# deepomicslab/PALACE

Measured on AMD Instinct MI355X. Metric: contigs/sec eref+generate_graph+matching, 1M-contig synth, 1/2/4/8 GPU, higher is better.
Workload: dtype u32

## Files before the change

palace_amd/csrc/common.hpp:

```cpp
#pragma once
#include <hip/hip_runtime.h>
#include <cstdarg>
#include <cstdint>
#include <cstdio>
#include <cstring>
#include <vector>

#include "../../include/palace_hip.h"

namespace palace {

void set_error(const char *fmt, ...);

#define PALACE_HIP_TRY(expr)                                                                    \
    do {                                                                                        \
        hipError_t e__ = (expr);                                                                \
        if (e__ != hipSuccess) {                                                                \
            palace::set_error("%s failed: %s (%s:%d)", #expr, hipGetErrorString(e__), __FILE__, \
                              __LINE__);                                                        \
            return PALACE_EHIP;                                                                 \
        }                                                                                       \
    } while (0)

#define PALACE_REQUIRE(cond, msg)                                  \
// ... 11 lines not shown

struct CoderMasks {
    uint32_t m[3][3];
};

struct Workspace {
    void *ptr = nullptr;
    size_t bytes = 0;
};

}

namespace palace {
struct MatchScratch;
void free_match_scratch(MatchScratch *m);
}

struct palace_ctx {
    int device = 0;
    hipStream_t stream = nullptr;
    bool owns_stream = true;
    hipEvent_t ev0 = nullptr, ev1 = nullptr;
    uint32_t key_buckets[4] = {~0u, ~0u, ~0u, ~0u};
    std::vector<hipEvent_t> marks;
    bool coder_set = false;
    palace::CoderMasks masks{};
    uint32_t *plane[3] = {nullptr, nullptr, nullptr};
    bool planes_external = false;
    bool want_final = false;
    bool final_only = false;
    bool table_clean = false;
    int64_t keys_counted = 0;
    const struct palace_eref_probe_index *probe_ix = nullptr;
    const struct palace_eref_probe_index *c0_hits_ix = nullptr;
    uint32_t hits_mask = 0;
    int probe_all_sets = 0;
    bool sent_scattered = false;
    int64_t scan_ref_lo = 0, scan_ref_hi = 0;
    const void *counts_ptr = nullptr;
    bool planeless = false;
    int count_mode = 0;
    int64_t bin_cap_override = 0;
    int64_t slab_override = 0;
    palace::Workspace ws;
    bool ws_grown = false;
    palace::Workspace pin;
    palace::MatchScratch *match_scratch = nullptr;
    int64_t graph_border = -1;
    const void *graph_border_cands = nullptr;
    int64_t graph_border_n = -1;
    int match_grid = 0;
    bool match_two_word_keys = false;
    int match_iters = 0;
    uint64_t *d_small = nullptr;
};

namespace palace {
int ensure_workspace(palace_ctx *ctx, size_t bytes);
int ensure_pinned(palace_ctx *ctx, size_t bytes);
int ensure_table(palace_ctx *ctx);
}
```

palace_amd/csrc/decomp.hip:

```cpp
#include "decomp.hpp"

#include <algorithm>

namespace palace {

namespace {

constexpr uint64_t kNoKey = ~0ull;
constexpr uint64_t kClosed = 0;
constexpr int kStampShift = 42;
constexpr int kPackedShift = 52, kPackedStamps = 1 << (64 - kPackedShift);
constexpr uint64_t kLenMask = (1ull << 40) - 1;


__device__ __forceinline__ uint64_t wave_incl_scan(uint64_t v, int lane)
{
#pragma unroll
    for (int d = 1; d < 64; d <<= 1) {
        const uint64_t u = __shfl_up(v, d);
        if (lane >= d) v += u;
    }
    return v;
}

constexpr int kMaxWaves = 16;

__device__ void scan_partials_body(const uint64_t *__restrict__ in, int64_t n, uint64_t *__restrict__ partials, int blk, int nblk)
{
    __shared__ uint64_t part[kMaxWaves];
    const int64_t chunk = (n + nblk - 1) / nblk;
    const int64_t a = min(n, static_cast<int64_t>(blk) * chunk), e = min(n, a + chunk);
    uint64_t s = 0;
    for (int64_t i = a + threadIdx.x; i < e; i += blockDim.x) s += in[i];
    const int lane = threadIdx.x & 63, waves = static_cast<int>(blockDim.x >> 6);
    s = wave_incl_scan(s, lane);
    if (lane == 63) part[threadIdx.x >> 6] = s;
    __syncthreads();
    if (threadIdx.x == 0) {
        uint64_t t = 0;
        for (int w = 0; w < waves; w++) t += part[w];
        partials[blk] = t;
    }
    __syncthreads();
}

__device__ void scan_prefix_body(uint64_t *__restrict__ partials, int n_parts, uint64_t *__restrict__ total)
{
    __shared__ uint64_t part[kMaxWaves];
    const int lane = threadIdx.x & 63, wv = threadIdx.x >> 6;
    const uint64_t x = static_cast<int>(threadIdx.x) < n_parts ? partials[threadIdx.x] : 0;
    const uint64_t incl = wave_incl_scan(x, lane);
    if (lane == 63) part[wv] = incl;
    __syncthreads();
    uint64_t before = 0;
    for (int w = 0; w < wv; w++) before += part[w];
    if (static_cast<int>(threadIdx.x) < n_parts) partials[threadIdx.x] = before + incl - x;
    if (threadIdx.x == blockDim.x - 1) *total = before + incl;
    __syncthreads();
}

__device__ void scan_apply_body(const uint64_t *__restrict__ in, uint64_t *__restrict__ out, int64_t n, const uint64_t *__restrict__ partials,
                                int blk, int nblk)
{
    __shared__ uint64_t part[kMaxWaves];
    const int64_t chunk = (n + nblk - 1) / nblk;
    const int64_t a = min(n, static_cast<int64_t>(blk) * chunk), e = min(n, a + chunk);
    const int lane = threadIdx.x & 63, wv = threadIdx.x >> 6, waves = static_cast<int>(blockDim.x >> 6);
    uint64_t carry = partials[blk];
    for (int64_t base = a; base < e; base += blockDim.x) {
        const int64_t i = base + threadIdx.x;
        const uint64_t x = i < e ? in[i] : 0;
        const uint64_t incl = wave_incl_scan(x, lane);
        if (lane == 63) part[wv] = incl;
        __syncthreads();
        uint64_t before = 0, all = 0;
        for (int w = 0; w < waves; w++) { if (w < wv) before += part[w]; all += part[w]; }
        if (i < e) out[i] = carry + before + incl - x;
        carry += all;
        __syncthreads();
    }
}

__global__ __launch_bounds__(kDecompBlock) void scan_partials_kernel(const uint64_t *__restrict__ in, const int32_t *__restrict__ n_dev,
                                                                     uint64_t *__restrict__ partials)
{
    scan_partials_body(in, *n_dev, partials, static_cast<int>(blockIdx.x), static_cast<int>(gridDim.x));
}
__global__ __launch_bounds__(kDecompBlock) void scan_prefix_kernel(uint64_t *__restrict__ partials, int n_parts, uint64_t *__restrict__ total)
{
    scan_prefix_body(partials, n_parts, total);
}
__global__ __launch_bounds__(kDecompBlock) void scan_apply_kernel(const uint64_t *__restrict__ in, uint64_t *__restrict__ out,
                                                                  const int32_t *__restrict__ n_dev, const uint64_t *__restrict__ partials)
{
    scan_apply_body(in, out, *n_dev, partials, static_cast<int>(blockIdx.x), static_cast<int>(gridDim.x));
}

struct Span { int tid, n; };
__device__ __forceinline__ Span whole_grid() { return Span{static_cast<int>(blockIdx.x * blockDim.x + threadIdx.x), static_cast<int>(gridDim.x * blockDim.x)}; }

__device__ void ph_init(const DecompBufs &b, Span T, int64_t comp_cap, int64_t vert_cap, int n_flags, int allow_packed)
{
    DecompState *st = b.st;
    const int V = st->V;
    for (int i = T.tid; i < V; i += T.n) { b.bo_hi[i] = kNoKey; b.bi_hi[i] = kNoKey; b.on_path[i] = 0; }
    for (int i = T.tid; i < n_flags; i += T.n) b.changed[i] = 0;
    if (T.tid == 0) {
        st->n_comp = 0; st->n_vert = 0; st->comp_cap = comp_cap; st->vert_cap = vert_cap;
        st->unsettled = 0; st->overflow = 0; st->bad = 0; st->dead = 0; st->scan_total = 0; st->alive_after = 0;
        st->packed = (allow_packed && b.kc && b.pack_bad && *b.pack_bad == 0) ? 1u : 0u;
        if (comp_cap >= 0) b.o_off[0] = 0;
    }
}

__device__ void ph_round_begin(const DecompBufs &b, Span T, int reset_left)
{
    const int V = b.st->V;
    if (!reset_left && b.st->dead) return;
    if (T.tid == 0) { b.st->alive_after = 0; if (reset_left) b.st->dead = 0; }
    const int64_t E = b.st->E;
    for (int64_t e = T.tid; e < E; e += T.n) b.done[e] = 0;
    const bool packed = b.st->packed != 0;
    for (int i = T.tid; i < V; i += T.n) {
        const int s = i >> 1;
        const int64_t l = reset_left ? 1 : b.left[s];
        if (reset_left && !(i & 1)) b.left[s] = 1;
        b.alive[i] = l > 0;
        b.next[i] = -1; b.prev[i] = -1;
        b.bo_hi[i] = b.bi_hi[i] = l > 0 ? kNoKey : kClosed;
        if (!packed) { b.bo_lo[i] = kNoKey; b.bo_lo[V + i] = kNoKey; b.bi_lo[i] = kNoKey; b.bi_lo[V + i] = kNoKey; }
        b.len_a[i] = 0;
    }
}

struct IterArgs {
    uint64_t stamp;
    uint64_t stamp_p;
    int parity;
    int prev_flag, flag;
    int unique_hi;
};


__device__ void ph_propose_hi(const DecompBufs &b, Span T, const IterArgs &a)
{
    if (b.st->dead) return;
    if (a.prev_flag >= 0 && !b.changed[a.prev_flag]) return;
    const int64_t E = b.st->E;
    const int V = b.st->V;
    const int other = (a.parity ^ 1) * V;
    const bool packed = b.st->packed != 0;
    for (int64_t e = T.tid; e < E; e += T.n) {
        if (b.done[e]) continue;
        const int u = b.src[e], v = b.dst[e];
        if (b.bi_hi[v] == kClosed) { b.done[e] = 1; continue; }
        const uint64_t k = packed ? (a.stamp_p | b.kc[e]) : (a.stamp | b.khi[e]);
        if (atomicMin(reinterpret_cast<unsigned long long *>(&b.bo_hi[u]), static_cast<unsigned long long>(k)) == kClosed) { b.done[e] = 1; continue; }
        atomicMin(reinterpret_cast<unsigned long long *>(&b.bi_hi[v]), static_cast<unsigned long long>(k));
        if (!a.unique_hi && !packed) { b.bo_lo[other + u] = kNoKey; b.bi_lo[other + v] = kNoKey; }
    }
}

__device__ void ph_propose_lo(const DecompBufs &b, Span T, const IterArgs &a)
{
    if (b.st->dead) return;
    if (a.prev_flag >= 0 && !b.changed[a.prev_flag]) return;
    if (b.st->packed) return;
    const int64_t E = b.st->E;
    const int mine = a.parity * b.st->V;
    for (int64_t e = T.tid; e < E; e += T.n) {
        if (b.done[e]) continue;
        const int u = b.src[e], v = b.dst[e];
        const uint64_t k = a.stamp | b.khi[e], lo = b.klo[e];
        if (b.bo_hi[u] == k) atomicMin(reinterpret_cast<unsigned long long *>(&b.bo_lo[mine + u]), static_cast<unsigned long long>(lo));
        if (b.bi_hi[v] == k) atomicMin(reinterpret_cast<unsigned long long *>(&b.bi_lo[mine + v]), static_cast<unsigned long long>(lo));
    }
}

__device__ void ph_commit_flag(const DecompBufs &b, Span T, const IterArgs &a, volatile unsigned int *took);
__device__ void ph_commit(const DecompBufs &b, Span T, const IterArgs &a)
{
    if (b.st->dead) return;
    if (a.prev_flag >= 0 && !b.changed[a.prev_flag]) return;
    ph_commit_flag(b, T, a, b.changed + a.flag);
}
__device__ void ph_commit_flag(const DecompBufs &b, Span T, const IterArgs &a, volatile unsigned int *took)
{
    bool any = false;
    const int64_t E = b.st->E;
    const int mine = a.parity * b.st->V;
    const bool packed = b.st->packed != 0;
    for (int64_t e = T.tid; e < E; e += T.n) {
        if (b.done[e]) continue;
        const int u = b.src[e], v = b.dst[e];
        const uint64_t k = packed ? (a.stamp_p | b.kc[e]) : (a.stamp | b.khi[e]);
        if (b.bo_hi[u] != k || b.bi_hi[v] != k) continue;
        const uint64_t lo = b.klo[e];
        if (!a.unique_hi && !packed && (b.bo_lo[mine + u] != lo || b.bi_lo[mine + v] != lo)) continue;
        b.next[u] = v; b.prev[v] = u;
        b.nhi[u] = b.khi[e]; b.nlo[u] = lo;
        b.bo_hi[u] = kClosed; b.bi_hi[v] = kClosed;
        b.done[e] = 1;
        any = true;
    }
    if (__syncthreads_or(any) && threadIdx.x == 0) *took = 1u;
}

__device__ void ph_heads(const DecompBufs &b, Span T, int round, int last_flag)
{
    DecompState *st = b.st;
    if (st->dead) return;
    if (T.tid == 0 && last_flag >= 0 && b.changed[last_flag]) st->unsettled = 1;
    const int V = st->V;
    for (int v = T.tid; v < V; v += T.n) {
        if (!b.alive[v] || b.prev[v] >= 0) continue;
        int len = 0, last = v;
        int64_t least = b.left[v >> 1];
        for (int x = v; x >= 0; x = b.next[x]) {
            b.on_path[x] = round + 1;
            last = x;
            len++;
            least = min(least, b.left[x >> 1]);
        }
        const int twin_first = last ^ 1;
        if (v > twin_first) continue;
        const int64_t uses = twin_first == v ? 2 : 1;
        b.len_a[v] = (1ull << 40) | static_cast<uint64_t>(len);
        b.pay[v] = max(static_cast<int64_t>(1), least / uses);
        b.kind[v] = 0;
        b.open_at[v] = 0;
    }
}

__device__ void ph_cycles(const DecompBufs &b, Span T, int round)
{
    const int V = b.st->V;
    if (b.st->dead) return;
    for (int v = T.tid; v < V; v += T.n) {
        if (!b.alive[v] || b.on_path[v] == round + 1) continue;
        int len = 1, twin_least = v ^ 1, worst = 0;
        uint64_t whi = b.nhi[v], wlo = b.nlo[v];
        int64_t least = b.left[v >> 1];
        bool first = true;
        for (int x = b.next[v]; x != v; x = b.next[x]) {
            if (x < v) { first = false; break; }
            twin_least = min(twin_least, x ^ 1);
            const uint64_t hi = b.nhi[x], lo = b.nlo[x];
            if (hi > whi || (hi == whi && lo > wlo)) { whi = hi; wlo = lo; worst = len; }
            least = min(least, b.left[x >> 1]);
            len++;
        }
        if (!first || v > twin_least) continue;
        const int64_t uses = twin_least == v ? 2 : 1;
        b.len_a[v] = (1ull << 40) | static_cast<uint64_t>(len);
        b.pay[v] = max(static_cast<int64_t>(1), least / uses);
        b.kind[v] = 1;
        b.open_at[v] = (worst + 1) % len;
    }
}

__device__ void ph_emit(const DecompBufs &b, Span T, int round, int64_t c0, int64_t v0)
{
    DecompState *st = b.st;
    const int V = st->V;
    if (st->dead) return;
    int64_t alive = 0;
    for (int v = T.tid; v < V; v += T.n) {
        const uint64_t la = b.len_a[v];
        if (!la) continue;
        const int64_t len = static_cast<int64_t>(la & kLenMask);
        const uint64_t p = b.pos[v];
        const int64_t c = c0 + static_cast<int64_t>(p >> 40), at = v0 + static_cast<int64_t>(p & kLenMask);
        const int64_t pay = b.pay[v];
        const bool room = c < st->comp_cap && at + len <= st->vert_cap;
        if (!room) st->overflow = 1;
        else { b.o_off[c] = at; b.o_kind[c] = b.kind[v]; b.o_iter[c] = round; b.o_open[c] = b.open_at[v]; }
        int x = v;
        int64_t still = 0;
        for (int64_t k = 0; k < len; k++) {
            if (room) b.o_verts[at + k] = 2 * b.orig[x >> 1] + (x & 1);
            const int64_t l = b.left[x >> 1];
            b.left[x >> 1] = max(static_cast<int64_t>(0), l - pay);
            still += l - pay > 0;
            x = b.next[x];
        }
        alive += still;
    }
    __shared__ unsigned long long wg_alive;
    if (threadIdx.x == 0) wg_alive = 0;
    __syncthreads();
    if (alive) atomicAdd(&wg_alive, static_cast<unsigned long long>(alive));
    __syncthreads();
    if (threadIdx.x == 0 && wg_alive) atomicAdd(reinterpret_cast<unsigned long long *>(&st->alive_after), wg_alive);
}


__global__ void dec_init_kernel(DecompBufs b, int64_t comp_cap, int64_t vert_cap, int n_flags, int allow_packed) { ph_init(b, whole_grid(), comp_cap, vert_cap, n_flags, allow_packed); }
__global__ void dec_round_begin_kernel(DecompBufs b, int reset_left) { ph_round_begin(b, whole_grid(), reset_left); }
__global__ void dec_propose_hi_kernel(DecompBufs b, IterArgs a) { ph_propose_hi(b, whole_grid(), a); }
__global__ void dec_propose_lo_kernel(DecompBufs b, IterArgs a) { ph_propose_lo(b, whole_grid(), a); }
__global__ void dec_commit_kernel(DecompBufs b, IterArgs a) { ph_commit(b, whole_grid(), a); }
__global__ void dec_heads_kernel(DecompBufs b, int round, int last_flag) { ph_heads(b, whole_grid(), round, last_flag); }
__global__ void dec_cycles_kernel(DecompBufs b, int round) { ph_cycles(b, whole_grid(), round); }
__global__ void dec_emit_kernel(DecompBufs b, int round) { ph_emit(b, whole_grid(), round, b.st->n_comp, b.st->n_vert); }

__global__ void dec_round_end_kernel(DecompBufs b)
{
    DecompState *st = b.st;
    if (blockIdx.x || threadIdx.x || st->dead) return;
    st->dead = st->alive_after == 0;
    st->n_comp += static_cast<int64_t>(st->scan_total >> 40);
    st->n_vert += static_cast<int64_t>(st->scan_total & kLenMask);
    if (st->n_comp <= st->comp_cap) b.o_off[st->n_comp] = st->n_vert;
}

size_t up256(size_t v) { return (v + 255) / 256 * 256; }

struct Carver {
    char *base;
    size_t used = 0;
    template <class T>
    T *take(size_t n)
    {
        T *p = base ? reinterpret_cast<T *>(base + used) : nullptr;
        used += up256(std::max<size_t>(1, n) * sizeof(T));
        return p;
    }
};

size_t carve_all(DecompBufs &b, char *base, int64_t s_cap, int64_t e_cap, int64_t comp_cap, int64_t vert_cap, int rounds, int iters)
{
    Carver c{base};
    const size_t S = static_cast<size_t>(std::max<int64_t>(1, s_cap)), V = 2 * S, E = static_cast<size_t>(std::max<int64_t>(1, e_cap));
    b.st = c.take<DecompState>(1);
    b.src = c.take<int32_t>(E); b.dst = c.take<int32_t>(E);
    b.khi = c.take<uint64_t>(E); b.klo = c.take<uint64_t>(E);
    b.done = c.take<uint8_t>(E);
    b.kc = c.take<uint64_t>(E);
    b.left = c.take<int64_t>(S); b.orig = c.take<int32_t>(S);
    b.next = c.take<int32_t>(V); b.prev = c.take<int32_t>(V); b.on_path = c.take<int32_t>(V); b.open_at = c.take<int32_t>(V);
    b.nhi = c.take<uint64_t>(V); b.nlo = c.take<uint64_t>(V);
    b.bo_hi = c.take<uint64_t>(V); b.bi_hi = c.take<uint64_t>(V);
    b.bo_lo = c.take<uint64_t>(2 * V); b.bi_lo = c.take<uint64_t>(2 * V);
    b.len_a = c.take<uint64_t>(V); b.pos = c.take<uint64_t>(V);
    b.pay = c.take<int64_t>(V);
    b.alive = c.take<uint8_t>(V); b.kind = c.take<uint8_t>(V);
    b.partials = c.take<uint64_t>(kDecompGrid + 1);
    b.changed = c.take<uint32_t>(static_cast<size_t>(rounds) * static_cast<size_t>(iters));
    b.o_off = c.take<int64_t>(static_cast<size_t>(comp_cap) + 1);
    b.o_verts = c.take<int32_t>(static_cast<size_t>(vert_cap));
    b.o_iter = c.take<int32_t>(static_cast<size_t>(comp_cap));
    b.o_open = c.take<int32_t>(static_cast<size_t>(comp_cap));
    b.o_kind = c.take<uint8_t>(static_cast<size_t>(comp_cap));
    return c.used;
}

}

size_t decomp_bytes(int64_t s_cap, int64_t e_cap, int64_t comp_cap, int64_t vert_cap, int rounds, int iters)
{
    DecompBufs tmp;
    return carve_all(tmp, nullptr, s_cap, e_cap, comp_cap, vert_cap, rounds, iters);
}

void decomp_carve(DecompBufs &b, char *base, int64_t s_cap, int64_t e_cap, int64_t comp_cap, int64_t vert_cap, int rounds, int iters)
{
    carve_all(b, base, s_cap, e_cap, comp_cap, vert_cap, rounds, iters);
}

int scan_u64(palace_ctx *ctx, const uint64_t *in, uint64_t *out, const int32_t *n_dev, uint64_t *partials, uint64_t *total_dev)
{
    hipLaunchKernelGGL(scan_partials_kernel, dim3(kDecompGrid), dim3(kDecompBlock), 0, ctx->stream, in, n_dev, partials);
    hipLaunchKernelGGL(scan_prefix_kernel, dim3(1), dim3(kDecompBlock), 0, ctx->stream, partials, kDecompGrid, total_dev);
    hipLaunchKernelGGL(scan_apply_kernel, dim3(kDecompGrid), dim3(kDecompBlock), 0, ctx->stream, in, out, n_dev, partials);
    PALACE_HIP_TRY(hipGetLastError());
    return PALACE_OK;
}

namespace {

const dim3 kBlock(kDecompBlock);
constexpr int kWideGridDefault = 2048;
inline dim3 wide_grid(const palace_ctx *ctx) { return dim3(ctx->match_grid > 0 ? ctx->match_grid : kWideGridDefault); }

void enqueue_iterations(palace_ctx *ctx, const DecompBufs &b, int first, int n, uint64_t *count, int flag0, bool unique_hi)
{
    for (int k = 0; k < n; k++) {
        IterArgs a{((1ull << 21) - 1 - *count) << kStampShift, static_cast<uint64_t>((kPackedStamps - 1 - *count) & (kPackedStamps - 1)) << kPackedShift,
                   (first + k) & 1, k ? flag0 + k - 1 : -1, flag0 + k, unique_hi ? 1 : 0};
        (*count)++;
        hipLaunchKernelGGL(dec_propose_hi_kernel, wide_grid(ctx), kBlock, 0, ctx->stream, b, a);
        if (!unique_hi) hipLaunchKernelGGL(dec_propose_lo_kernel, wide_grid(ctx), kBlock, 0, ctx->stream, b, a);
        hipLaunchKernelGGL(dec_commit_kernel, wide_grid(ctx), kBlock, 0, ctx->stream, b, a);
    }
}

int enqueue_read_off(palace_ctx *ctx, const DecompBufs &b, int round, int last_flag)
{
    hipLaunchKernelGGL(dec_heads_kernel, wide_grid(ctx), kBlock, 0, ctx->stream, b, round, last_flag);
    hipLaunchKernelGGL(dec_cycles_kernel, wide_grid(ctx), kBlock, 0, ctx->stream, b, round);
    int rc = scan_u64(ctx, b.len_a, b.pos, &b.st->V, b.partials, &b.st->scan_total);
    if (rc) return rc;
    hipLaunchKernelGGL(dec_emit_kernel, wide_grid(ctx), kBlock, 0, ctx->stream, b, round);
    hipLaunchKernelGGL(dec_round_end_kernel, dim3(1), dim3(64), 0, ctx->stream, b);
    PALACE_HIP_TRY(hipGetLastError());
    return PALACE_OK;
}

}

int decomp_begin(palace_ctx *ctx, const DecompBufs &b, int rounds, int64_t comp_cap, int64_t vert_cap)
{
    PALACE_REQUIRE(rounds >= 1 && rounds <= kMaxRounds, "round count out of range");
    static_assert(kDecompGrid <= kDecompBlock, "scan_prefix_kernel scans the block sums with one workgroup");
    const int allow_packed = !ctx->match_two_word_keys && static_cast<int64_t>(rounds) * kMaxIters < kPackedStamps ? 1 : 0;
    hipLaunchKernelGGL(dec_init_kernel, wide_grid(ctx), kBlock, 0, ctx->stream, b, comp_cap, vert_cap, rounds * kMaxIters, allow_packed);
    PALACE_HIP_TRY(hipGetLastError());
    return PALACE_OK;
}

int decomp_rounds(palace_ctx *ctx, const DecompBufs &b, int t0, int t1, int rounds, int aggressive, int iters, bool unique_hi,
                  uint64_t *count)
{
    PALACE_REQUIRE(0 <= t0 && t0 <= t1 && t1 <= rounds && rounds <= kMaxRounds && iters >= 1 && iters <= kMaxIters, "round / iteration count out of range");
    for (int t = t0; t < t1; t++) {
        hipLaunchKernelGGL(dec_round_begin_kernel, wide_grid(ctx), kBlock, 0, ctx->stream, b, (aggressive && t == rounds - 1) ? 1 : 0);
        enqueue_iterations(ctx, b, 0, iters, count, t * kMaxIters, unique_hi);
        int rc = enqueue_read_off(ctx, b, t, t * kMaxIters + iters - 1);
        if (rc) return rc;
    }
    PALACE_HIP_TRY(hipGetLastError());
    return PALACE_OK;
}

int decomp_run_checked(palace_ctx *ctx, const DecompBufs &b, int rounds, int aggressive, bool unique_hi, int64_t comp_cap,
                       int64_t vert_cap, int64_t max_iterations)
{
    PALACE_REQUIRE(rounds >= 1 && rounds <= kMaxRounds, "round count out of range");
    constexpr int kBatch = 16;
    hipLaunchKernelGGL(dec_init_kernel, wide_grid(ctx), kBlock, 0, ctx->stream, b, comp_cap, vert_cap, kBatch, 0);
    uint64_t count = 0;
    for (int t = 0; t < rounds; t++) {
        hipLaunchKernelGGL(dec_round_begin_kernel, wide_grid(ctx), kBlock, 0, ctx->stream, b, (aggressive && t == rounds - 1) ? 1 : 0);
        for (int first = 0;; first += kBatch) {
            PALACE_HIP_TRY(hipMemsetAsync(b.changed, 0, kBatch * sizeof(uint32_t), ctx->stream));
            enqueue_iterations(ctx, b, first, kBatch, &count, 0, unique_hi);
            uint32_t last = 0;
            PALACE_HIP_TRY(hipMemcpyAsync(&last, b.changed + kBatch - 1, sizeof last, hipMemcpyDeviceToHost, ctx->stream));
            PALACE_HIP_TRY(hipStreamSynchronize(ctx->stream));
            if (!last) break;
            if (static_cast<int64_t>(count) > max_iterations || count + kBatch >= (1ull << 21)) {
                set_error("matching: no fixed point after %llu iterations", static_cast<unsigned long long>(count));
                return PALACE_ESTATE;
            }
        }
        PALACE_HIP_TRY(hipMemsetAsync(b.changed, 0, kBatch * sizeof(uint32_t), ctx->stream));
        int rc = enqueue_read_off(ctx, b, t, kBatch - 1);
        if (rc) return rc;
    }
    return PALACE_OK;
}

int decomp_group(palace_ctx *ctx, const DecompBufs &b, DecompRun &run, int rounds, int aggressive, bool unique_hi)
{
    const int first = kFirstGroupRounds;
    const int t0 = run.next_round, t1 = std::min(rounds, t0 + (t0 == 0 ? first : kRoundsPerGroup));
    for (int t = t0; t < t1; t++) {
        const int iters = ctx->match_iters > 0 ? std::min(ctx->match_iters, kMaxIters) : (t == 0 ? kFirstRoundIters : kLaterRoundIters);
        int rc = decomp_rounds(ctx, b, t, t + 1, rounds, aggressive, iters, unique_hi, &run.count);
        if (rc) return rc;
    }
    run.next_round = t1;
    return PALACE_OK;
}

int decomp_finish(palace_ctx *ctx, const DecompBufs &b, DecompRun &run, int rounds, int aggressive, bool unique_hi, int64_t comp_cap,
                  int64_t vert_cap, int64_t max_iterations, DecompState *h_state, const std::function<int()> &reset_left)
{
    for (;;) {
        PALACE_HIP_TRY(hipMemcpyAsync(h_state, b.st, sizeof *h_state, hipMemcpyDeviceToHost, ctx->stream));
        PALACE_HIP_TRY(hipStreamSynchronize(ctx->stream));
        if (h_state->unsettled) {
            int rc = reset_left();
            if (rc) return rc;
            rc = decomp_run_checked(ctx, b, rounds, aggressive, unique_hi, comp_cap, vert_cap, max_iterations);
            if (rc) return rc;
            PALACE_HIP_TRY(hipMemcpyAsync(h_state, b.st, sizeof *h_state, hipMemcpyDeviceToHost, ctx->stream));
            PALACE_HIP_TRY(hipStreamSynchronize(ctx->stream));
            return PALACE_OK;
        }
        if (run.next_round >= rounds) return PALACE_OK;
        if (h_state->alive_after == 0) {
            if (!aggressive) return PALACE_OK;
            run.next_round = rounds - 1;
        }
        int rc = decomp_group(ctx, b, run, rounds, aggressive, unique_hi);
        if (rc) return rc;
    }
}

}
```

palace_amd/csrc/decomp.hpp:

```cpp
#pragma once
#include <functional>

#include "common.hpp"

struct palace_match_result {
    int64_t n = 0;
    int64_t *off = nullptr;
    int32_t *verts = nullptr, *iter = nullptr, *open_at = nullptr;
    uint8_t *kind = nullptr;
    uint64_t *bare = nullptr;
    int64_t n_bare = 0;
    bool borrowed = false;
    ~palace_match_result();
};

namespace palace {

constexpr int kDecompGrid = 256;
constexpr int kDecompBlock = 256;
constexpr int kMaxRounds = 1024;
constexpr int kMaxIters = 64;

struct DecompState {
    int32_t S, V;
    int64_t E;
    int64_t n_comp, n_vert;
    int64_t comp_cap, vert_cap;
    uint32_t unsettled;
    uint32_t overflow;
    uint32_t bad;
    uint32_t dead;
    uint32_t packed;
    uint64_t scan_total;
    int64_t alive_after;
};

struct DecompBufs {
    DecompState *st = nullptr;
    int32_t *src = nullptr, *dst = nullptr;
    uint64_t *khi = nullptr, *klo = nullptr;
    uint8_t *done = nullptr;
    uint64_t *kc = nullptr;
    const uint32_t *pack_bad = nullptr;
    int64_t *left = nullptr;
    int32_t *orig = nullptr;
    int32_t *next = nullptr, *prev = nullptr, *on_path = nullptr, *open_at = nullptr;
    uint64_t *nhi = nullptr, *nlo = nullptr;
    uint64_t *bo_hi = nullptr, *bi_hi = nullptr;
    uint64_t *bo_lo = nullptr, *bi_lo = nullptr;
    uint64_t *len_a = nullptr, *pos = nullptr;
    int64_t *pay = nullptr;
    uint8_t *alive = nullptr, *kind = nullptr;
    uint64_t *partials = nullptr;
    uint32_t *changed = nullptr;
    int64_t *o_off = nullptr;
    int32_t *o_verts = nullptr, *o_iter = nullptr, *o_open = nullptr;
    uint8_t *o_kind = nullptr;
};

size_t decomp_bytes(int64_t s_cap, int64_t e_cap, int64_t comp_cap, int64_t vert_cap, int rounds, int iters);
void decomp_carve(DecompBufs &b, char *base, int64_t s_cap, int64_t e_cap, int64_t comp_cap, int64_t vert_cap, int rounds, int iters);
constexpr int kFirstRoundIters = 7, kLaterRoundIters = 4, kRoundsPerGroup = 5, kFirstGroupRounds = 5;
int decomp_begin(palace_ctx *ctx, const DecompBufs &b, int rounds, int64_t comp_cap, int64_t vert_cap);
int decomp_rounds(palace_ctx *ctx, const DecompBufs &b, int t0, int t1, int rounds, int aggressive, int iters, bool unique_hi,
                  uint64_t *count);

struct DecompRun { int next_round = 0; uint64_t count = 0; };
int decomp_group(palace_ctx *ctx, const DecompBufs &b, DecompRun &run, int rounds, int aggressive, bool unique_hi);
int decomp_finish(palace_ctx *ctx, const DecompBufs &b, DecompRun &run, int rounds, int aggressive, bool unique_hi, int64_t comp_cap,
                  int64_t vert_cap, int64_t max_iterations, DecompState *h_state, const std::function<int()> &reset_left);

int decomp_run_checked(palace_ctx *ctx, const DecompBufs &b, int rounds, int aggressive, bool unique_hi, int64_t comp_cap,
                       int64_t vert_cap, int64_t max_iterations);

int scan_u64(palace_ctx *ctx, const uint64_t *in, uint64_t *out, const int32_t *n_dev, uint64_t *partials, uint64_t *total_dev);

}
```

palace_amd/csrc/match.hip:

```cpp
#include "common.hpp"
#include "decomp.hpp"
#include <algorithm>
#include <map>
#include <memory>
#include <mutex>
#include <numeric>
#include <thread>

namespace palace {

constexpr int32_t kNone = -1;

struct MatchArgs {
    int32_t n_vertices;
    int64_t n_arcs;
    const int32_t *src, *dst;
    const int64_t *out_off, *in_off;
    const int32_t *out_arcs, *in_arcs;
    const uint8_t *alive;
    int32_t *next, *prev, *next_arc, *want_out, *want_in;
    unsigned int *changed;
};

__global__ void match_propose_kernel(MatchArgs a)
// ... 282 lines not shown
    pair.clear(); w.clear(); m_pair.clear(); m_w.clear();
    pair.reserve(2 * n_edges); w.reserve(2 * n_edges);
    for (int64_t e = 0; e < n_edges; e++) {
        const palace_graph_edge &x = edges[e];
        const int64_t tot = static_cast<int64_t>(x.counts[0]) + x.counts[1] + x.counts[2] + x.counts[3];
        if (tot < min_count) continue;
        PALACE_REQUIRE(x.left >= 0 && x.left < n_segs && x.right >= 0 && x.right < n_segs, "edge endpoint out of range");
        const uint64_t u = 2ull * x.left + (x.oL & 1), v = 2ull * x.right + (x.oR & 1);
        pair.push_back(u * V + v); w.push_back(tot);
        if ((v ^ 1) != u) { pair.push_back((v ^ 1) * V + (u ^ 1)); w.push_back(tot); }
    }
    const size_t n = pair.size();
    perm.resize(n); tmp.resize(n);
    std::iota(perm.begin(), perm.end(), 0u);
    radix_by(pair, perm, tmp);
    m_pair.reserve(n); m_w.reserve(n);
    for (size_t i = 0; i < n; i++) {
        if (!m_pair.empty() && m_pair.back() == pair[perm[i]]) m_w.back() += w[perm[i]];
        else { m_pair.push_back(pair[perm[i]]); m_w.push_back(w[perm[i]]); }
    }
    const size_t m = m_pair.size();
    int64_t w_max = 0;
    for (int64_t x : m_w) w_max = std::max(w_max, x);
    m_cls.resize(m); m_wkey.resize(m);
    for (size_t i = 0; i < m; i++) {
        const uint64_t u = m_pair[i] / V, v = m_pair[i] % V;
        m_cls[i] = std::min(m_pair[i], (v ^ 1) * V + (u ^ 1));
        m_wkey[i] = static_cast<uint64_t>(w_max - m_w[i]);
    }
    perm.resize(m); tmp.resize(m);
    std::iota(perm.begin(), perm.end(), 0u);
    radix_by(m_cls, perm, tmp);
    radix_by(m_wkey, perm, tmp);
    for (size_t i = 0; i < m; i++) {
        const uint64_t p = m_pair[perm[i]];
        src[i] = static_cast<int32_t>(p / V); dst[i] = static_cast<int32_t>(p % V); weight[i] = m_w[perm[i]];
    }
    *n_arcs_out = static_cast<int64_t>(m);
    return PALACE_OK;
}

int palace_match_set_option(palace_ctx *ctx, const char *name, int64_t value)
{
    PALACE_REQUIRE(ctx && name, "null argument");
    if (!std::strcmp(name, "iters_per_round")) {
        PALACE_REQUIRE(value >= 0 && value <= palace::kMaxIters, "iters_per_round out of range");
        ctx->match_iters = static_cast<int>(value);
    } else if (!std::strcmp(name, "one_word_keys")) {
        PALACE_REQUIRE(value == 0 || value == 1, "one_word_keys must be 0 or 1");
        ctx->match_two_word_keys = value == 0;
    } else if (!std::strcmp(name, "decomp_grid")) {
        PALACE_REQUIRE(value >= 0 && value <= 65536, "decomp_grid out of range");
        ctx->match_grid = static_cast<int>(value);
    } else {
        palace::set_error("palace_match_set_option: unknown option '%s'", name);
        return PALACE_EINVAL;
    }
    return PALACE_OK;
}

int palace_match_decompose(palace_ctx *ctx, int32_t n_segs, const int64_t *copies, int64_t n_arcs,
                           const int32_t *src, const int32_t *dst, int32_t iterations, int32_t aggressive,
                           palace_match_result **out)
{
    return palace_match_decompose_ex(ctx, n_segs, copies, n_arcs, src, dst, iterations, aggressive, 0, out);
}

int palace_match_decompose_ex(palace_ctx *ctx, int32_t n_segs, const int64_t *copies, int64_t n_arcs,
                              const int32_t *src, const int32_t *dst, int32_t iterations, int32_t aggressive,
                              int32_t compact, palace_match_result **out)
{
    PALACE_REQUIRE(ctx && out && n_segs >= 0 && n_arcs >= 0 && iterations >= 1, "bad argument");
    PALACE_REQUIRE(n_segs == 0 || copies, "null copies");
    PALACE_REQUIRE(n_arcs == 0 || (src && dst), "null arc arrays");
    PALACE_REQUIRE(n_segs < (1 << 30) && n_arcs < (1ll << 31), "graph too large for int32 ids");
    PALACE_HIP_TRY(hipSetDevice(ctx->device));
    const int32_t V = 2 * n_segs;
    for (int64_t e = 0; e < n_arcs; e++)
        PALACE_REQUIRE(src[e] >= 0 && src[e] < V && dst[e] >= 0 && dst[e] < V, "arc endpoint out of range");
    if (!ctx->match_scratch) ctx->match_scratch = new palace::MatchScratch();
    palace::MatchScratch &ms = *ctx->match_scratch;
    palace::Borrowed<std::vector<int32_t>> b_new(ms.new_id), b_old(ms.old_id), b_ssrc(ms.ssrc), b_sdst(ms.sdst);
    palace::Borrowed<std::vector<int64_t>> b_sc(ms.sub_copies);
    auto &new_id = b_new.v, &old_id = b_old.v, &ssrc = b_ssrc.v, &sdst = b_sdst.v;
    auto &sub_copies = b_sc.v;
    SubResult &sub = ms.sub;
    const size_t n_words = (static_cast<size_t>(n_segs) + 63) / 64;
    palace::Borrowed<std::vector<uint64_t>> b_bits(ms.has_arc);
    auto &has_arc = b_bits.v;
    has_arc.assign(n_words, 0);
    for (int64_t e = 0; e < n_arcs; e++) {
        const int32_t a = src[e] >> 1, b = dst[e] >> 1;
        has_arc[a >> 6] |= 1ull << (a & 63);
        has_arc[b >> 6] |= 1ull << (b & 63);
    }
    new_id.resize(n_words + 1);
    old_id.clear();
    for (size_t w = 0; w < n_words; w++) {
        new_id[w] = static_cast<int32_t>(old_id.size());
        for (uint64_t x = has_arc[w]; x; x &= x - 1) old_id.push_back(static_cast<int32_t>(w * 64 + __builtin_ctzll(x)));
    }
    new_id[n_words] = static_cast<int32_t>(old_id.size());
    auto is_sub = [&](int32_t sg) { return (has_arc[sg >> 6] >> (sg & 63)) & 1ull; };
    auto sub_rank = [&](int32_t sg) {
        if (sg >= n_segs) return new_id[n_words];
        return new_id[sg >> 6] + __builtin_popcountll(has_arc[sg >> 6] & ((1ull << (sg & 63)) - 1));
// ... 131 lines not shown
```

Before: 112.8 million.

## Run decomposition rounds in one persistent kernel with software grid barriers

Replaces the per-phase kernel launches of each matching round (propose, commit, heads, cycles, scan, emit, round end) with a single resident kernel that loops over rounds and iterations and separates phases with an atomic-counter grid barrier. Shared state is accessed through relaxed agent-scope atomics. The goal is to remove per-launch dispatch overhead and inter-kernel gaps for the many small phases. In exchange the grid is limited to one workgroup per CU, and a barrier timeout path can fail the run if workgroups are not co-resident. It also adds a diagnostic dispatch-only build mode.

```diff
diff --git a/palace_amd/csrc/common.hpp b/palace_amd/csrc/common.hpp
--- a/palace_amd/csrc/common.hpp
+++ b/palace_amd/csrc/common.hpp
@@ -87,6 +87,8 @@
     int match_grid = 0;
     bool match_two_word_keys = false;
     int match_iters = 0;
+    bool match_resident = true;
+    int match_resident_grid = 0;
     uint64_t *d_small = nullptr;
 };
 
diff --git a/palace_amd/csrc/decomp.hip b/palace_amd/csrc/decomp.hip
--- a/palace_amd/csrc/decomp.hip
+++ b/palace_amd/csrc/decomp.hip
@@ -1,6 +1,8 @@
 #include "decomp.hpp"
 
 #include <algorithm>
+#include <cstdlib>
+#include <type_traits>
 
 namespace palace {
 
@@ -13,6 +15,19 @@
 constexpr uint64_t kLenMask = (1ull << 40) - 1;
 
 
+template <bool R, class T>
+__device__ __forceinline__ void put(T *p, std::common_type_t<T> v)
+{
+    if constexpr (R) __hip_atomic_store(p, v, __ATOMIC_RELAXED, __HIP_MEMORY_SCOPE_AGENT);
+    else *p = v;
+}
+template <bool R, class T>
+__device__ __forceinline__ T get(const T *p)
+{
+    if constexpr (R) return __hip_atomic_load(p, __ATOMIC_RELAXED, __HIP_MEMORY_SCOPE_AGENT);
+    else return *p;
+}
+
 __device__ __forceinline__ uint64_t wave_incl_scan(uint64_t v, int lane)
 {
 #pragma unroll
@@ -25,6 +40,7 @@
 
 constexpr int kMaxWaves = 16;
 
+template <bool R = false>
 __device__ void scan_partials_body(const uint64_t *__restrict__ in, int64_t n, uint64_t *__restrict__ partials, int blk, int nblk)
 {
     __shared__ uint64_t part[kMaxWaves];
@@ -39,11 +55,12 @@
     if (threadIdx.x == 0) {
         uint64_t t = 0;
         for (int w = 0; w < waves; w++) t += part[w];
-        partials[blk] = t;
-    }
-    __syncthreads();
-}
-
+        put<R>(&partials[blk], t);
+    }
+    __syncthreads();
+}
+
+template <bool R = false>
 __device__ void scan_prefix_body(uint64_t *__restrict__ partials, int n_parts, uint64_t *__restrict__ total)
 {
     __shared__ uint64_t part[kMaxWaves];
@@ -54,11 +71,12 @@
     __syncthreads();
     uint64_t before = 0;
     for (int w = 0; w < wv; w++) before += part[w];
-    if (static_cast<int>(threadIdx.x) < n_parts) partials[threadIdx.x] = before + incl - x;
-    if (threadIdx.x == blockDim.x - 1) *total = before + incl;
-    __syncthreads();
-}
-
+    if (static_cast<int>(threadIdx.x) < n_parts) put<R>(&partials[threadIdx.x], before + incl - x);
+    if (threadIdx.x == blockDim.x - 1) put<R>(total, before + incl);
+    __syncthreads();
+}
+
+template <bool R = false>
 __device__ void scan_apply_body(const uint64_t *__restrict__ in, uint64_t *__restrict__ out, int64_t n, const uint64_t *__restrict__ partials,
                                 int blk, int nblk)
 {
@@ -75,7 +93,7 @@
         __syncthreads();
         uint64_t before = 0, all = 0;
         for (int w = 0; w < waves; w++) { if (w < wv) before += part[w]; all += part[w]; }
-        if (i < e) out[i] = carry + before + incl - x;
+        if (i < e) put<R>(&out[i], carry + before + incl - x);
         carry += all;
         __syncthreads();
     }
@@ -108,28 +126,30 @@
     if (T.tid == 0) {
         st->n_comp = 0; st->n_vert = 0; st->comp_cap = comp_cap; st->vert_cap = vert_cap;
         st->unsettled = 0; st->overflow = 0; st->bad = 0; st->dead = 0; st->scan_total = 0; st->alive_after = 0;
+        st->bar_count = 0; st->bar_exit = 0; st->bar_timeout = 0;
         st->packed = (allow_packed && b.kc && b.pack_bad && *b.pack_bad == 0) ? 1u : 0u;
         if (comp_cap >= 0) b.o_off[0] = 0;
     }
 }
 
+template <bool R = false>
 __device__ void ph_round_begin(const DecompBufs &b, Span T, int reset_left)
 {
     const int V = b.st->V;
-    if (!reset_left && b.st->dead) return;
-    if (T.tid == 0) { b.st->alive_after = 0; if (reset_left) b.st->dead = 0; }
+    if (!reset_left && get<R>(&b.st->dead)) return;
+    if (T.tid == 0) { put<R>(&b.st->alive_after, static_cast<int64_t>(0)); if (reset_left) put<R>(&b.st->dead, 0u); }
     const int64_t E = b.st->E;
     for (int64_t e = T.tid; e < E; e += T.n) b.done[e] = 0;
     const bool packed = b.st->packed != 0;
     for (int i = T.tid; i < V; i += T.n) {
         const int s = i >> 1;
         const int64_t l = reset_left ? 1 : b.left[s];
-        if (reset_left && !(i & 1)) b.left[s] = 1;
+        if (reset_left && !(i & 1)) put<R>(&b.left[s], static_cast<int64_t>(1));
         b.alive[i] = l > 0;
-        b.next[i] = -1; b.prev[i] = -1;
-        b.bo_hi[i] = b.bi_hi[i] = l > 0 ? kNoKey : kClosed;
-        if (!packed) { b.bo_lo[i] = kNoKey; b.bo_lo[V + i] = kNoKey; b.bi_lo[i] = kNoKey; b.bi_lo[V + i] = kNoKey; }
-        b.len_a[i] = 0;
+        put<R>(&b.next[i], -1); put<R>(&b.prev[i], -1);
+        put<R>(&b.bo_hi[i], l > 0 ? kNoKey : kClosed); put<R>(&b.bi_hi[i], l > 0 ? kNoKey : kClosed);
+        if (!packed) { put<R>(&b.bo_lo[i], kNoKey); put<R>(&b.bo_lo[V + i], kNoKey); put<R>(&b.bi_lo[i], kNoKey); put<R>(&b.bi_lo[V + i], kNoKey); }
+        put<R>(&b.len_a[i], static_cast<uint64_t>(0));
     }
 }
 
@@ -142,10 +162,11 @@
 };
 
 
+template <bool R = false>
 __device__ void ph_propose_hi(const DecompBufs &b, Span T, const IterArgs &a)
 {
-    if (b.st->dead) return;
-    if (a.prev_flag >= 0 && !b.changed[a.prev_flag]) return;
+    if (get<R>(&b.st->dead)) return;
+    if (a.prev_flag >= 0 && !get<R>(&b.changed[a.prev_flag])) return;
     const int64_t E = b.st->E;
     const int V = b.st->V;
     const int other = (a.parity ^ 1) * V;
@@ -157,14 +178,15 @@
         const uint64_t k = packed ? (a.stamp_p | b.kc[e]) : (a.stamp | b.khi[e]);
         if (atomicMin(reinterpret_cast<unsigned long long *>(&b.bo_hi[u]), static_cast<unsigned long long>(k)) == kClosed) { b.done[e] = 1; continue; }
         atomicMin(reinterpret_cast<unsigned long long *>(&b.bi_hi[v]), static_cast<unsigned long long>(k));
-        if (!a.unique_hi && !packed) { b.bo_lo[other + u] = kNoKey; b.bi_lo[other + v] = kNoKey; }
-    }
-}
-
+        if (!a.unique_hi && !packed) { put<R>(&b.bo_lo[other + u], kNoKey); put<R>(&b.bi_lo[other + v], kNoKey); }
+    }
+}
+
+template <bool R = false>
 __device__ void ph_propose_lo(const DecompBufs &b, Span T, const IterArgs &a)
 {
-    if (b.st->dead) return;
-    if (a.prev_flag >= 0 && !b.changed[a.prev_flag]) return;
+    if (get<R>(&b.st->dead)) return;
+    if (a.prev_flag >= 0 && !get<R>(&b.changed[a.prev_flag])) return;
     if (b.st->packed) return;
     const int64_t E = b.st->E;
     const int mine = a.parity * b.st->V;
@@ -177,13 +199,16 @@
     }
 }
 
+template <bool R>
 __device__ void ph_commit_flag(const DecompBufs &b, Span T, const IterArgs &a, volatile unsigned int *took);
+template <bool R = false>
 __device__ void ph_commit(const DecompBufs &b, Span T, const IterArgs &a)
 {
-    if (b.st->dead) return;
-    if (a.prev_flag >= 0 && !b.changed[a.prev_flag]) return;
-    ph_commit_flag(b, T, a, b.changed + a.flag);
-}
+    if (get<R>(&b.st->dead)) return;
+    if (a.prev_flag >= 0 && !get<R>(&b.changed[a.prev_flag])) return;
+    ph_commit_flag<R>(b, T, a, b.changed + a.flag);
+}
+template <bool R>
 __device__ void ph_commit_flag(const DecompBufs &b, Span T, const IterArgs &a, volatile unsigned int *took)
 {
     bool any = false;
@@ -197,27 +222,31 @@
         if (b.bo_hi[u] != k || b.bi_hi[v] != k) continue;
         const uint64_t lo = b.klo[e];
         if (!a.unique_hi && !packed && (b.bo_lo[mine + u] != lo || b.bi_lo[mine + v] != lo)) continue;
-        b.next[u] = v; b.prev[v] = u;
-        b.nhi[u] = b.khi[e]; b.nlo[u] = lo;
-        b.bo_hi[u] = kClosed; b.bi_hi[v] = kClosed;
+        put<R>(&b.next[u], v); put<R>(&b.prev[v], u);
+        put<R>(&b.nhi[u], b.khi[e]); put<R>(&b.nlo[u], lo);
+        put<R>(&b.bo_hi[u], kClosed); put<R>(&b.bi_hi[v], kClosed);
         b.done[e] = 1;
         any = true;
     }
-    if (__syncthreads_or(any) && threadIdx.x == 0) *took = 1u;
-}
-
+    if (__syncthreads_or(any) && threadIdx.x == 0) {
+        if constexpr (R) put<R>(const_cast<unsigned int *>(took), 1u);
+        else *took = 1u;
+    }
+}
+
+template <bool R = false>
 __device__ void ph_heads(const DecompBufs &b, Span T, int round, int last_flag)
 {
     DecompState *st = b.st;
-    if (st->dead) return;
-    if (T.tid == 0 && last_flag >= 0 && b.changed[last_flag]) st->unsettled = 1;
+    if (get<R>(&st->dead)) return;
+    if (T.tid == 0 && last_flag >= 0 && get<R>(&b.changed[last_flag])) put<R>(&st->unsettled, 1u);
     const int V = st->V;
     for (int v = T.tid; v < V; v += T.n) {
         if (!b.alive[v] || b.prev[v] >= 0) continue;
         int len = 0, last = v;
         int64_t least = b.left[v >> 1];
         for (int x = v; x >= 0; x = b.next[x]) {
-            b.on_path[x] = round + 1;
+            put<R>(&b.on_path[x], round + 1);
             last = x;
             len++;
             least = min(least, b.left[x >> 1]);
@@ -225,17 +254,18 @@
         const int twin_first = last ^ 1;
         if (v > twin_first) continue;
         const int64_t uses = twin_first == v ? 2 : 1;
-        b.len_a[v] = (1ull << 40) | static_cast<uint64_t>(len);
+        put<R>(&b.len_a[v], (1ull << 40) | static_cast<uint64_t>(len));
         b.pay[v] = max(static_cast<int64_t>(1), least / uses);
         b.kind[v] = 0;
         b.open_at[v] = 0;
     }
 }
 
+template <bool R = false>
 __device__ void ph_cycles(const DecompBufs &b, Span T, int round)
 {
     const int V = b.st->V;
-    if (b.st->dead) return;
+    if (get<R>(&b.st->dead)) return;
     for (int v = T.tid; v < V; v += T.n) {
         if (!b.alive[v] || b.on_path[v] == round + 1) continue;
         int len = 1, twin_least = v ^ 1, worst = 0;
@@ -252,18 +282,19 @@
         }
         if (!first || v > twin_least) continue;
         const int64_t uses = twin_least == v ? 2 : 1;
-        b.len_a[v] = (1ull << 40) | static_cast<uint64_t>(len);
+        put<R>(&b.len_a[v], (1ull << 40) | static_cast<uint64_t>(len));
         b.pay[v] = max(static_cast<int64_t>(1), least / uses);
         b.kind[v] = 1;
         b.open_at[v] = (worst + 1) % len;
     }
 }
 
+template <bool R = false>
 __device__ void ph_emit(const DecompBufs &b, Span T, int round, int64_t c0, int64_t v0)
 {
     DecompState *st = b.st;
     const int V = st->V;
-    if (st->dead) return;
+    if (get<R>(&st->dead)) return;
     int64_t alive = 0;
     for (int v = T.tid; v < V; v += T.n) {
         const uint64_t la = b.len_a[v];
@@ -273,14 +304,14 @@
         const int64_t c = c0 + static_cast<int64_t>(p >> 40), at = v0 + static_cast<int64_t>(p & kLenMask);
         const int64_t pay = b.pay[v];
         const bool room = c < st->comp_cap && at + len <= st->vert_cap;
-        if (!room) st->overflow = 1;
+        if (!room) put<R>(&st->overflow, 1u);
         else { b.o_off[c] = at; b.o_kind[c] = b.kind[v]; b.o_iter[c] = round; b.o_open[c] = b.open_at[v]; }
         int x = v;
         int64_t still = 0;
         for (int64_t k = 0; k < len; k++) {
             if (room) b.o_verts[at + k] = 2 * b.orig[x >> 1] + (x & 1);
             const int64_t l = b.left[x >> 1];
-            b.left[x >> 1] = max(static_cast<int64_t>(0), l - pay);
+            put<R>(&b.left[x >> 1], max(static_cast<int64_t>(0), l - pay));
             still += l - pay > 0;
             x = b.next[x];
         }
@@ -304,15 +335,121 @@
 __global__ void dec_cycles_kernel(DecompBufs b, int round) { ph_cycles(b, whole_grid(), round); }
 __global__ void dec_emit_kernel(DecompBufs b, int round) { ph_emit(b, whole_grid(), round, b.st->n_comp, b.st->n_vert); }
 
-__global__ void dec_round_end_kernel(DecompBufs b)
+template <bool R = false>
+__device__ void ph_round_end(const DecompBufs &b)
 {
     DecompState *st = b.st;
-    if (blockIdx.x || threadIdx.x || st->dead) return;
-    st->dead = st->alive_after == 0;
-    st->n_comp += static_cast<int64_t>(st->scan_total >> 40);
-    st->n_vert += static_cast<int64_t>(st->scan_total & kLenMask);
-    if (st->n_comp <= st->comp_cap) b.o_off[st->n_comp] = st->n_vert;
-}
+    if (blockIdx.x || threadIdx.x || get<R>(&st->dead)) return;
+    const uint64_t total = get<R>(&st->scan_total);
+    const int64_t n_comp = st->n_comp + static_cast<int64_t>(total >> 40), n_vert = st->n_vert + static_cast<int64_t>(total & kLenMask);
+    put<R>(&st->dead, get<R>(&st->alive_after) == 0 ? 1u : 0u);
+    put<R>(&st->n_comp, n_comp);
+    put<R>(&st->n_vert, n_vert);
+    if (n_comp <= st->comp_cap) b.o_off[n_comp] = n_vert;
+}
+__global__ void dec_round_end_kernel(DecompBufs b) { ph_round_end(b); }
+
+constexpr unsigned kBarrierPolls = 1u << 20;
+
+struct GridBarrier {
+    DecompState *st;
+    unsigned target;
+};
+
+__device__ __forceinline__ bool grid_barrier(GridBarrier &g)
+{
+    __shared__ unsigned ok;
+    asm volatile("s_waitcnt vmcnt(0)" ::: "memory");
+    __syncthreads();
+    g.target += gridDim.x;
+    if (threadIdx.x == 0) {
+        __hip_atomic_fetch_add(&g.st->bar_count, 1u, __ATOMIC_RELAXED, __HIP_MEMORY_SCOPE_AGENT);
+        unsigned good = 1;
+        for (unsigned polls = 0; __hip_atomic_load(&g.st->bar_count, __ATOMIC_RELAXED, __HIP_MEMORY_SCOPE_AGENT) < g.target; polls++) {
+            if (polls >= kBarrierPolls) __hip_atomic_store(&g.st->bar_timeout, 1u, __ATOMIC_RELAXED, __HIP_MEMORY_SCOPE_AGENT);
+            if (polls >= kBarrierPolls || __hip_atomic_load(&g.st->bar_timeout, __ATOMIC_RELAXED, __HIP_MEMORY_SCOPE_AGENT)) { good = 0; break; }
+            __builtin_amdgcn_s_sleep(16);
+        }
+        __builtin_amdgcn_fence(__ATOMIC_ACQUIRE, "agent");
+        asm volatile("s_waitcnt vmcnt(0)" ::: "memory");
+        ok = good;
+    }
+    __syncthreads();
+    return ok != 0;
+}
+
+struct ResidentArgs {
+    int t0, t1;
+    int rounds, aggressive, unique_hi;
+    int iters_first, iters_later;
+    uint64_t count;
+};
+
+#define DEC_BARRIER() do { if (!grid_barrier(bar)) return; } while (0)
+
+__global__ __launch_bounds__(kDecompBlock) void dec_rounds_resident_kernel(DecompBufs b, ResidentArgs g)
+{
+    constexpr bool R = true;
+    const Span T = whole_grid();
+    const int blk = static_cast<int>(blockIdx.x), nblk = static_cast<int>(gridDim.x);
+    DecompState *st = b.st;
+    GridBarrier bar{st, 0u};
+    uint64_t count = g.count;
+    for (int t = g.t0; t < g.t1; t++) {
+        const int iters = t == 0 ? g.iters_first : g.iters_later;
+        const int reset_left = (g.aggressive && t == g.rounds - 1) ? 1 : 0;
+        const uint64_t count0 = count;
+        count += static_cast<uint64_t>(iters);
+        if (!reset_left && get<R>(&st->dead)) continue;
+        const bool two_pass = !g.unique_hi && !get<R>(&st->packed);
+        ph_round_begin<R>(b, T, reset_left);
+        DEC_BARRIER();
+        for (int k = 0; k < iters; k++) {
+            const uint64_t c = count0 + static_cast<uint64_t>(k);
+            const IterArgs a{((1ull << 21) - 1 - c) << kStampShift, static_cast<uint64_t>((kPackedStamps - 1 - c) & (kPackedStamps - 1)) << kPackedShift,
+                             k & 1, k ? t * kMaxIters + k - 1 : -1, t * kMaxIters + k, g.unique_hi};
+            if (k && !get<R>(&b.changed[a.prev_flag])) break;
+            ph_propose_hi<R>(b, T, a);
+            DEC_BARRIER();
+            if (two_pass) { ph_propose_lo<R>(b, T, a); DEC_BARRIER(); }
+            ph_commit<R>(b, T, a);
+            DEC_BARRIER();
+        }
+        ph_heads<R>(b, T, t, t * kMaxIters + iters - 1);
+        DEC_BARRIER();
+        ph_cycles<R>(b, T, t);
+        DEC_BARRIER();
+        const int64_t V = st->V;
+        scan_partials_body<R>(b.len_a, V, b.partials, blk, nblk);
+        DEC_BARRIER();
+        if (blk == 0) scan_prefix_body<R>(b.partials, nblk, &st->scan_total);
+        DEC_BARRIER();
+        scan_apply_body<R>(b.len_a, b.pos, V, b.partials, blk, nblk);
+        DEC_BARRIER();
+        ph_emit<R>(b, T, t, get<R>(&st->n_comp), get<R>(&st->n_vert));
+        DEC_BARRIER();
+        ph_round_end<R>(b);
+        DEC_BARRIER();
+    }
+    __syncthreads();
+    if (threadIdx.x == 0 && __hip_atomic_fetch_add(&st->bar_exit, 1u, __ATOMIC_RELAXED, __HIP_MEMORY_SCOPE_AGENT) == gridDim.x - 1) {
+        __hip_atomic_store(&st->bar_count, 0u, __ATOMIC_RELAXED, __HIP_MEMORY_SCOPE_AGENT);
+        __hip_atomic_store(&st->bar_exit, 0u, __ATOMIC_RELAXED, __HIP_MEMORY_SCOPE_AGENT);
+    }
+}
+#undef DEC_BARRIER
+
+#ifdef PALACE_DIAG_DISPATCH_ONLY
+__global__ void dec_nop_kernel(DecompBufs) {}
+bool g_diag_dead = false;
+#define DEC_LAUNCH(kernel, grid, block, stream, b, ...)                                                        \
+    do {                                                                                                       \
+        if (g_diag_dead) hipLaunchKernelGGL(dec_nop_kernel, grid, block, 0, stream, b);                        \
+        else hipLaunchKernelGGL(kernel, grid, block, 0, stream, b, ##__VA_ARGS__);                             \
+    } while (0)
+#else
+#define DEC_LAUNCH(kernel, grid, block, stream, b, ...) hipLaunchKernelGGL(kernel, grid, block, 0, stream, b, ##__VA_ARGS__)
+#endif
 
 size_t up256(size_t v) { return (v + 255) / 256 * 256; }
 
@@ -389,20 +526,29 @@
         IterArgs a{((1ull << 21) - 1 - *count) << kStampShift, static_cast<uint64_t>((kPackedStamps - 1 - *count) & (kPackedStamps - 1)) << kPackedShift,
                    (first + k) & 1, k ? flag0 + k - 1 : -1, flag0 + k, unique_hi ? 1 : 0};
         (*count)++;
-        hipLaunchKernelGGL(dec_propose_hi_kernel, wide_grid(ctx), kBlock, 0, ctx->stream, b, a);
-        if (!unique_hi) hipLaunchKernelGGL(dec_propose_lo_kernel, wide_grid(ctx), kBlock, 0, ctx->stream, b, a);
-        hipLaunchKernelGGL(dec_commit_kernel, wide_grid(ctx), kBlock, 0, ctx->stream, b, a);
+        DEC_LAUNCH(dec_propose_hi_kernel, wide_grid(ctx), kBlock, ctx->stream, b, a);
+        if (!unique_hi) DEC_LAUNCH(dec_propose_lo_kernel, wide_grid(ctx), kBlock, ctx->stream, b, a);
+        DEC_LAUNCH(dec_commit_kernel, wide_grid(ctx), kBlock, ctx->stream, b, a);
     }
 }
 
 int enqueue_read_off(palace_ctx *ctx, const DecompBufs &b, int round, int last_flag)
 {
-    hipLaunchKernelGGL(dec_heads_kernel, wide_grid(ctx), kBlock, 0, ctx->stream, b, round, last_flag);
-    hipLaunchKernelGGL(dec_cycles_kernel, wide_grid(ctx), kBlock, 0, ctx->stream, b, round);
-    int rc = scan_u64(ctx, b.len_a, b.pos, &b.st->V, b.partials, &b.st->scan_total);
-    if (rc) return rc;
-    hipLaunchKernelGGL(dec_emit_kernel, wide_grid(ctx), kBlock, 0, ctx->stream, b, round);
-    hipLaunchKernelGGL(dec_round_end_kernel, dim3(1), dim3(64), 0, ctx->stream, b);
+    DEC_LAUNCH(dec_heads_kernel, wide_grid(ctx), kBlock, ctx->stream, b, round, last_flag);
+    DEC_LAUNCH(dec_cycles_kernel, wide_grid(ctx), kBlock, ctx->stream, b, round);
+#ifdef PALACE_DIAG_DISPATCH_ONLY
+    if (g_diag_dead) {
+        hipLaunchKernelGGL(dec_nop_kernel, dim3(kDecompGrid), dim3(kDecompBlock), 0, ctx->stream, b);
+        hipLaunchKernelGGL(dec_nop_kernel, dim3(1), dim3(kDecompBlock), 0, ctx->stream, b);
+        hipLaunchKernelGGL(dec_nop_kernel, dim3(kDecompGrid), dim3(kDecompBlock), 0, ctx->stream, b);
+    } else
+#endif
+    {
+        int rc = scan_u64(ctx, b.len_a, b.pos, &b.st->V, b.partials, &b.st->scan_total);
+        if (rc) return rc;
+    }
+    DEC_LAUNCH(dec_emit_kernel, wide_grid(ctx), kBlock, ctx->stream, b, round);
+    DEC_LAUNCH(dec_round_end_kernel, dim3(1), dim3(64), ctx->stream, b);
     PALACE_HIP_TRY(hipGetLastError());
     return PALACE_OK;
 }
@@ -416,6 +562,11 @@
     const int allow_packed = !ctx->match_two_word_keys && static_cast<int64_t>(rounds) * kMaxIters < kPackedStamps ? 1 : 0;
     hipLaunchKernelGGL(dec_init_kernel, wide_grid(ctx), kBlock, 0, ctx->stream, b, comp_cap, vert_cap, rounds * kMaxIters, allow_packed);
     PALACE_HIP_TRY(hipGetLastError());
+#ifdef PALACE_DIAG_DISPATCH_ONLY
+    static int begins = 0;
+    const char *live = getenv("PALACE_DIAG_LIVE_BEGINS");
+    g_diag_dead = ++begins > (live ? atoi(live) : 0);
+#endif
     return PALACE_OK;
 }
 
@@ -424,7 +575,7 @@
 {
     PALACE_REQUIRE(0 <= t0 && t0 <= t1 && t1 <= rounds && rounds <= kMaxRounds && iters >= 1 && iters <= kMaxIters, "round / iteration count out of range");
     for (int t = t0; t < t1; t++) {
-        hipLaunchKernelGGL(dec_round_begin_kernel, wide_grid(ctx), kBlock, 0, ctx->stream, b, (aggressive && t == rounds - 1) ? 1 : 0);
+        DEC_LAUNCH(dec_round_begin_kernel, wide_grid(ctx), kBlock, ctx->stream, b, (aggressive && t == rounds - 1) ? 1 : 0);
         enqueue_iterations(ctx, b, 0, iters, count, t * kMaxIters, unique_hi);
         int rc = enqueue_read_off(ctx, b, t, t * kMaxIters + iters - 1);
         if (rc) return rc;
@@ -461,10 +612,41 @@
     return PALACE_OK;
 }
 
+int resident_grid(palace_ctx *ctx)
+{
+    if (!ctx->match_resident_grid) {
+        int per_cu = 0, cus = 0;
+        if (hipOccupancyMaxActiveBlocksPerMultiprocessor(&per_cu, dec_rounds_resident_kernel, kDecompBlock, 0) != hipSuccess ||
+            hipDeviceGetAttribute(&cus, hipDeviceAttributeMultiprocessorCount, ctx->device) != hipSuccess || per_cu < 1 || cus < 1)
+            ctx->match_resident_grid = -1;
+        else
+            ctx->match_resident_grid = std::min(cus, kDecompGrid);
+    }
+    if (ctx->match_resident_grid < 0) return 0;
+    return ctx->match_grid > 0 ? std::min(ctx->match_grid, ctx->match_resident_grid) : ctx->match_resident_grid;
+}
+
 int decomp_group(palace_ctx *ctx, const DecompBufs &b, DecompRun &run, int rounds, int aggressive, bool unique_hi)
 {
     const int first = kFirstGroupRounds;
     const int t0 = run.next_round, t1 = std::min(rounds, t0 + (t0 == 0 ? first : kRoundsPerGroup));
+    const int grid = ctx->match_resident ? resident_grid(ctx) : 0;
+#ifdef PALACE_DIAG_DISPATCH_ONLY
+    if (false)
+#else
+    if (grid > 0 && t0 < t1)
+#endif
+    {
+        PALACE_REQUIRE(0 <= t0 && t1 <= rounds && rounds <= kMaxRounds, "round count out of range");
+        static_assert(kDecompGrid <= kDecompBlock, "the in-kernel scan's prefix step is one workgroup's");
+        const int fixed = ctx->match_iters > 0 ? std::min(ctx->match_iters, kMaxIters) : 0;
+        const ResidentArgs g{t0, t1, rounds, aggressive, unique_hi ? 1 : 0, fixed ? fixed : kFirstRoundIters, fixed ? fixed : kLaterRoundIters, run.count};
+        hipLaunchKernelGGL(dec_rounds_resident_kernel, dim3(grid), kBlock, 0, ctx->stream, b, g);
+        PALACE_HIP_TRY(hipGetLastError());
+        for (int t = t0; t < t1; t++) run.count += static_cast<uint64_t>(t == 0 ? g.iters_first : g.iters_later);
+        run.next_round = t1;
+        return PALACE_OK;
+    }
     for (int t = t0; t < t1; t++) {
         const int iters = ctx->match_iters > 0 ? std::min(ctx->match_iters, kMaxIters) : (t == 0 ? kFirstRoundIters : kLaterRoundIters);
         int rc = decomp_rounds(ctx, b, t, t + 1, rounds, aggressive, iters, unique_hi, &run.count);
@@ -480,6 +662,10 @@
     for (;;) {
         PALACE_HIP_TRY(hipMemcpyAsync(h_state, b.st, sizeof *h_state, hipMemcpyDeviceToHost, ctx->stream));
         PALACE_HIP_TRY(hipStreamSynchronize(ctx->stream));
+        if (h_state->bar_timeout) {
+            set_error("matching: the resident rounds kernel gave up at a grid barrier (its workgroups were not all resident in time)");
+            return PALACE_ESTATE;
+        }
         if (h_state->unsettled) {
             int rc = reset_left();
             if (rc) return rc;
diff --git a/palace_amd/csrc/decomp.hpp b/palace_amd/csrc/decomp.hpp
--- a/palace_amd/csrc/decomp.hpp
+++ b/palace_amd/csrc/decomp.hpp
@@ -33,6 +33,7 @@
     uint32_t packed;
     uint64_t scan_total;
     int64_t alive_after;
+    uint32_t bar_count, bar_exit, bar_timeout, bar_pad;
 };
 
 struct DecompBufs {
diff --git a/palace_amd/csrc/match.hip b/palace_amd/csrc/match.hip
--- a/palace_amd/csrc/match.hip
+++ b/palace_amd/csrc/match.hip
@@ -358,6 +358,9 @@
     } else if (!std::strcmp(name, "decomp_grid")) {
         PALACE_REQUIRE(value >= 0 && value <= 65536, "decomp_grid out of range");
         ctx->match_grid = static_cast<int>(value);
+    } else if (!std::strcmp(name, "resident_rounds")) {
+        PALACE_REQUIRE(value == 0 || value == 1, "resident_rounds must be 0 or 1");
+        ctx->match_resident = value == 1;
     } else {
         palace::set_error("palace_match_set_option: unknown option '%s'", name);
         return PALACE_EINVAL;
```

New measurement: 98.88 million, median of 2. -12.3%, worse.
